# yuzhou42/disinfect-slam

Measured on AMD Instinct MI355X. Metric: TSDF integrate frames/s (640x480 depth+label, 5mm voxel), higher is better.
Workload: dtype f32

## Files before the change

### disinfect-slam_amd/csrc/tsdf_block.h

```cpp
#pragma once

#include "tsdf_device.h"

namespace tsdf {

__device__ __forceinline__ int lane_id() { return threadIdx.x & 63; }

__device__ __forceinline__ float wave_min(float v) {
#pragma unroll
  for (int o = 32; o > 0; o >>= 1) v = fminf(v, __shfl_xor(v, o, 64));
  return v;
}
__device__ __forceinline__ float wave_min_u(float v) {
  v = fminf(v, __int_as_float(__builtin_amdgcn_update_dpp(0, __float_as_int(v), 0xB1, 0xF, 0xF, false)));
  v = fminf(v, __int_as_float(__builtin_amdgcn_update_dpp(0, __float_as_int(v), 0x4E, 0xF, 0xF, false)));
  v = fminf(v, __int_as_float(__builtin_amdgcn_update_dpp(0, __float_as_int(v), 0x141, 0xF, 0xF, false)));
  v = fminf(v, __int_as_float(__builtin_amdgcn_update_dpp(0, __float_as_int(v), 0x140, 0xF, 0xF, false)));
  const int x = __float_as_int(v);
  return fminf(fminf(__int_as_float(__builtin_amdgcn_readlane(x, 0)), __int_as_float(__builtin_amdgcn_readlane(x, 16))),
               fminf(__int_as_float(__builtin_amdgcn_readlane(x, 32)), __int_as_float(__builtin_amdgcn_readlane(x, 48))));
}
__device__ __forceinline__ int wave_sum(int v) {
#pragma unroll
  for (int o = 32; o > 0; o >>= 1) v += __shfl_xor(v, o, 64);
  return v;
}
__device__ __forceinline__ int wave_incl_scan(int v) {
  const int l = lane_id();
#pragma unroll
  for (int o = 1; o < 64; o <<= 1) {
    const int n = __shfl_up(v, o, 64);
    if (l >= o) v += n;
  }
  return v;
}
template <int NW = 0>
__device__ __forceinline__ int block_excl_scan(int v, int* scratch, int* total) {
  const int w = threadIdx.x >> 6, nw = NW ? NW : blockDim.x >> 6;
  const int incl = wave_incl_scan(v);
  if (lane_id() == 63) scratch[w] = incl;
  __syncthreads();
  int before = 0, tot = 0;
#pragma unroll
  for (int i = 0; i < nw; ++i) {
// ... 210 lines not shown
```

### disinfect-slam_amd/csrc/tsdf_device.h

```cpp
#pragma once

#include <hip/hip_runtime.h>
#include <stdint.h>


namespace tsdf {

constexpr int kBlockLenBits = 3;
constexpr int kBlockLen = 8;
constexpr int kBlockVolume = 512;
constexpr int kBlockVolumeBits = 9;
constexpr int kNumBucketBits = 21;
constexpr uint32_t kNumBucket = 1u << kNumBucketBits;
constexpr uint32_t kBucketMask = kNumBucket - 1;
constexpr uint32_t kNumEntry = kNumBucket * 2;
constexpr uint32_t kEntryMask = kNumEntry - 1;
constexpr uint32_t kOccWords = kNumEntry / 64;
constexpr int kBlockBytes = kBlockVolume * 12;
constexpr int kProbOffset = kBlockVolume * 4;
constexpr int kRgbwOffset = kBlockVolume * 8;
constexpr uint32_t kNewKeyCap = 1u << 17;
constexpr int kMaxDdaSamples = 6;
constexpr int64_t kMaxOrderRange = 8192ll * 1024;
constexpr int kResolveThreads = 1024;
// ... 128 lines not shown


__device__ __forceinline__ int32_t round_quot_i(float a, float b, float rb) {
  const float q = a * rb;
  const float h = __builtin_copysignf(0.5f, q);
  const int32_t i1 = f2i(__builtin_fmaf(q, 1.0f + 0x1p-20f, h));
  const int32_t i2 = f2i(__builtin_fmaf(q, 1.0f - 0x1p-20f, h));
  if (__builtin_expect(i1 == i2 && fabsf(b) < 0x1p100f, 1)) return i1;
  return f2i(roundf(a / b));
}
__device__ __forceinline__ uint32_t round_quot_u8(float a, float b, float rb) {
  return (uint32_t)min(255, max(0, round_quot_i(a, b, rb)));
}

typedef float v2f __attribute__((ext_vector_type(2)));
__device__ __forceinline__ v2f v2(float a, float b) {
  v2f r;
  r.x = a;
  r.y = b;
  return r;
}
__device__ __forceinline__ v2f vfma(v2f a, v2f b, v2f c) { return __builtin_elementwise_fma(a, b, c); }

__device__ __forceinline__ void round_quot_i2(v2f a, v2f b, v2f rb, bool act0, bool act1,
                                              int32_t& o0, int32_t& o1) {
  const v2f q = a * rb;
  const v2f h = v2(__builtin_copysignf(0.5f, q.x), __builtin_copysignf(0.5f, q.y));
  const v2f f1 = vfma(q, v2(1.0f + 0x1p-20f, 1.0f + 0x1p-20f), h);
  const v2f f2 = vfma(q, v2(1.0f - 0x1p-20f, 1.0f - 0x1p-20f), h);
  o0 = f2i(f1.x);
  o1 = f2i(f1.y);
  if (__builtin_expect(act0 && !(o0 == f2i(f2.x) && fabsf(b.x) < 0x1p100f), 0))
    o0 = f2i(roundf(a.x / b.x));
  if (__builtin_expect(act1 && !(o1 == f2i(f2.y) && fabsf(b.y) < 0x1p100f), 0))
    o1 = f2i(roundf(a.y / b.y));
}

__device__ __forceinline__ v2f quot_const2(v2f a, float b, float rb, bool act0, bool act1) {
  const v2f q = a * rb;
  const v2f r = vfma(-q, v2(b, b), a);
  v2f o = vfma(r, v2(rb, rb), q);
  const float fa0 = fabsf(a.x), fq0 = fabsf(q.x), fa1 = fabsf(a.y), fq1 = fabsf(q.y);
  if (__builtin_expect(act0 && !(fa0 > 0x1p-60f && fa0 < 0x1p60f && fq0 > 0x1p-60f && fq0 < 0x1p60f), 0))
    o.x = a.x / b;
  if (__builtin_expect(act1 && !(fa1 > 0x1p-60f && fa1 < 0x1p60f && fq1 > 0x1p-60f && fq1 < 0x1p60f), 0))
    o.y = a.y / b;
  return o;
}

__device__ __forceinline__ void round_quot_pos2(v2f a, v2f b, v2f rb, bool act0, bool act1,
                                                int32_t& o0, int32_t& o1) {
  const v2f q = a * rb;
  const v2f f1 = vfma(q, v2(1.0f + 0x1p-20f, 1.0f + 0x1p-20f), v2(0.5f, 0.5f));
  const v2f f2 = vfma(q, v2(1.0f - 0x1p-20f, 1.0f - 0x1p-20f), v2(0.5f, 0.5f));
  o0 = f2i(f1.x);
  o1 = f2i(f1.y);
  if (__builtin_expect(act0 && o0 != f2i(f2.x), 0)) o0 = f2i(roundf(a.x / b.x));
  if (__builtin_expect(act1 && o1 != f2i(f2.y), 0)) o1 = f2i(roundf(a.y / b.y));
}

__device__ __forceinline__ v2f div_pair(v2f a, v2f b, v2f y, bool act0, bool act1) {
  const v2f e = vfma(-b, y, v2(1.0f, 1.0f));
  const v2f y1 = vfma(e, y, y);
  const v2f q = a * y1;
  const v2f r = vfma(-b, q, a);
  const v2f q1 = vfma(r, y1, q);
  const v2f r1 = vfma(-b, q1, a);
  v2f o = vfma(r1, y1, q1);
  const float fa0 = fabsf(a.x), fb0 = fabsf(b.x), fa1 = fabsf(a.y), fb1 = fabsf(b.y);
  if (__builtin_expect(act0 && !(fa0 >= 0x1p-40f && fa0 <= 0x1p40f && fb0 >= 0x1p-40f && fb0 <= 0x1p40f), 0))
    o.x = a.x / b.x;
  if (__builtin_expect(act1 && !(fa1 >= 0x1p-40f && fa1 <= 0x1p40f && fb1 >= 0x1p-40f && fb1 <= 0x1p40f), 0))
    o.y = a.y / b.y;
  return o;
}

constexpr float kSemQ[9] = {0x1.555554p-2f,  -0x1.fffffcp-3f, 0x1.999d5ap-3f,  -0x1.555b4ap-3f, 0x1.23d21ap-3f,
                            -0x1.fcf4c6p-4f, 0x1.dea282p-4f,  -0x1.d635bcp-4f, 0x1.1d8ea4p-4f};
constexpr float kSemE[6] = {0x1p-1f, 0x1.555556p-3f, 0x1.5554eap-5f, 0x1.1110e0p-7f, 0x1.6d4316p-10f,
                            0x1.a124e4p-13f};
constexpr float kSemLn2Hi = 0x1.62e4p-1f;
constexpr float kSemLn2Lo = 0x1.7f7d1cp-20f;
constexpr float kSemInvLn2 = 0x1.715476p+0f;
constexpr float kSemSqrtHalf = 0x1.6a09e6p-1f;

__device__ __forceinline__ float sem_log_reduce(float x, float& dk) {
  const bool sub = x < 0x1p-126f;
  const uint32_t ix = __float_as_uint(sub ? x * 0x1p24f : x);
  const int32_t k = (int32_t)(ix - 0x3f3504f3u) >> 23;
  dk = (float)(sub ? k - 24 : k);
  return __uint_as_float(ix - ((uint32_t)k << 23)) - 1.0f;
}
__device__ __forceinline__ v2f sem_log_core2(v2f f, v2f dk) {
  v2f q = v2(kSemQ[8], kSemQ[8]);
#pragma unroll
  for (int i = 7; i >= 0; --i) q = vfma(q, f, v2(kSemQ[i], kSemQ[i]));
// ... 211 lines not shown
  for (int i = 0; i < 8; ++i) {
    const bool v = voxel_visible(P, (int16_t)(x + ((i >> 0) & 1) * (kBlockLen - 1)),
                                 (int16_t)(y + ((i >> 1) & 1) * (kBlockLen - 1)),
                                 (int16_t)(z + ((i >> 2) & 1) * (kBlockLen - 1)));
    if (Full)
      vis = vis && v;
    else
      vis = vis || v;
  }
  return vis;
}

__device__ __forceinline__ f3 pixel_ray(const FrameParams& P, int x, int y) {
  f3 pc;
  pc.x = P.ifx * (float)x + P.icx * 1.0f;
  pc.y = P.ify * (float)y + P.icy * 1.0f;
  pc.z = 1.0f;
  return pc;
}
__device__ __forceinline__ float pixel_w_new(const FrameParams& P, float d) {
  return (1.0f - quot_const(d, P.max_depth, P.inv_max_depth)) * 4.0f;
}

}
```

### disinfect-slam_amd/csrc/tsdf_fuse.hip

```cpp
#include "tsdf_block.h"
#include "tsdf_kernels.h"
#include "tsdf_resolve.h"
#include "tsdf_ingest.h"

namespace tsdf {

__device__ __forceinline__ float comp(const float4& v, int j) {
  return j == 0 ? v.x : j == 1 ? v.y : j == 2 ? v.z : v.w;
}
__device__ __forceinline__ void setc(float4& v, int j, float f) {
  if (j == 0) v.x = f; else if (j == 1) v.y = f; else if (j == 2) v.z = f; else v.w = f;
}
__device__ __forceinline__ uint32_t compu(const uint4& v, int j) {
  return j == 0 ? v.x : j == 1 ? v.y : j == 2 ? v.z : v.w;
}
__device__ __forceinline__ void setu(uint4& v, int j, uint32_t f) {
  if (j == 0) v.x = f; else if (j == 1) v.y = f; else if (j == 2) v.z = f; else v.w = f;
}

__device__ __forceinline__ void frame_end(const EngineDev& D) {
  lds_barrier();
  if (threadIdx.x == 0) {
    D.ctr->total_visible += (unsigned long long)D.ctr->n_vis;
    D.ctr->total_updated += D.ctr->last_updated;
// ... 159 lines not shown
  const int16_t ax0 = (int16_t)(r.x << kBlockLenBits), ay = (int16_t)((r.y << kBlockLenBits) + ry),
                az = (int16_t)((r.z << kBlockLenBits) + rz);
  const float fy = (float)ay * P.voxel, fz = (float)az * P.voxel;
  const float qx = P.cq.x, qy = P.cq.y, qz = P.cq.z, qw = P.cq.w;
  const float qx_fz = qx * fz, qx_fy = qx * fy;
  float uvx = qy * fz - qz * fy;
  uvx += uvx;
  const float w_uvx = qw * uvx, qz_uvx = qz * uvx, qy_uvx = qy * uvx;
#pragma unroll
  for (int k = 0; k < 2; ++k) {
    const v2f wx = v2((float)(int16_t)(ax0 + rx0 + 2 * k), (float)(int16_t)(ax0 + rx0 + 2 * k + 1)) * P.voxel;
    v2f uvy = qz * wx - qx_fz;
    v2f uvz = qx_fy - qy * wx;
    uvy += uvy;
    uvz += uvz;
    const v2f cx = qy * uvz - qz * uvy;
    const v2f cy = qz_uvx - qx * uvz;
    const v2f cz = qx * uvy - qy_uvx;
    const v2f pcx = ((wx + w_uvx) + cx) + P.ct.x;
    const v2f pcy = ((fy + qw * uvy) + cy) + P.ct.y;
    const v2f pcz = ((fz + qw * uvz) + cz) + P.ct.z;
    const v2f hx = P.fx * pcx + P.cx * pcz;
    const v2f hy = P.fy * pcy + P.cy * pcz;
    const v2f rz = v2(__builtin_amdgcn_rcpf(pcz.x), __builtin_amdgcn_rcpf(pcz.y));
    int u0, u1, v0, v1;
    round_quot_i2(hx, pcz, rz, true, true, u0, u1);
    round_quot_i2(hy, pcz, rz, true, true, v0, v1);
    hzs[k] = pcz;
    const int uu[2] = {u0, u1}, vv[2] = {v0, v1};
#pragma unroll
    for (int e = 0; e < 2; ++e) {
      const int j = 2 * k + e;
      inb[j] = uu[e] >= 0 && uu[e] < P.W && vv[e] >= 0 && vv[e] < P.H;
      const int img = inb[j] ? vv[e] * P.W + uu[e] : 0;
      if (Raw) {
        pc[j] = (uint32_t)P.rgb[3 * img] | ((uint32_t)P.rgb[3 * img + 1] << 8) |
                ((uint32_t)P.rgb[3 * img + 2] << 16);
        px[j] = make_float4(P.depth[img], P.ht ? P.ht[img] : 1.0f, P.lt ? P.lt[img] : 1.0f,
                            __int_as_float((uu[e] & 0xFFFF) | (vv[e] << 16)));
      } else {
        px[j] = D.pixA[P.pix_off + img];
        pc[j] = D.pixC[P.pix_off + img];
      }
    }
  }
}

template <bool Raw>
__device__ __forceinline__ void update_issue(const EngineDev& D, const FrameParams& P, const VisRec& r, int lane,
                                             int hf, UpdState& S) {
// ... 28 lines not shown
    bool pf0, pf1;
    if (Raw) {
      const int w0 = __float_as_int(px[j0].w), w1 = __float_as_int(px[j1].w);
      const f3 r0 = pixel_ray(P, w0 & 0xFFFF, w0 >> 16);
      const f3 r1 = pixel_ray(P, w1 & 0xFFFF, w1 >> 16);
      rng = v2(sqrtf(dot3(r0, r0)), sqrtf(dot3(r1, r1)));
      w_new = v2(pixel_w_new(P, d.x), pixel_w_new(P, d.y));
      lnh = sem_logf2(v2(px[j0].y, px[j1].y));
      lnl = sem_logf2(v2(px[j0].z, px[j1].z));
      pf0 = sem_pixel_fast(px[j0].y, px[j0].z, d.x, P.max_depth);
      pf1 = sem_pixel_fast(px[j1].y, px[j1].z, d.y, P.max_depth);
    } else {
      rng = v2(fabsf(px[j0].y), fabsf(px[j1].y));
      pf0 = px[j0].y > 0.0f;
      pf1 = px[j1].y > 0.0f;
      lnh = v2(px[j0].z, px[j1].z);
      lnl = v2(px[j0].w, px[j1].w);
    }
    const uint32_t n0 = pc[j0], n1 = pc[j1];
    const v2f sdf = rng * (d - hzs[k]);
    const bool a0 = inb[j0] && !(d.x == 0 || d.x > P.max_depth) && sdf.x > neg_trunc;
    const bool a1 = inb[j1] && !(d.y == 0 || d.y > P.max_depth) && sdf.y > neg_trunc;
    if (a0 || a1) {
      if (!Raw) w_new = (v2(1.0f, 1.0f) - quot_const2(d, P.max_depth, P.inv_max_depth, a0, a1)) * v2(4.0f, 4.0f);
      v2f tn = quot_const2(sdf, P.trunc, P.inv_trunc, a0, a1);
      tn = v2(fminf(1.0f, tn.x), fminf(1.0f, tn.y));
      const uint32_t o0 = compu(cw, j0), o1 = compu(cw, j1);
      const v2f w_old = v2((float)(o0 >> 24), (float)(o1 >> 24));
      const v2f wc = w_old + w_new;
      const v2f iwc = v2(__builtin_amdgcn_rcpf(wc.x), __builtin_amdgcn_rcpf(wc.y));
      uint32_t c0 = 0, c1 = 0;
#pragma unroll
      for (int ch = 0; ch < 3; ++ch) {
        const v2f num = v2((float)((o0 >> (8 * ch)) & 0xFF), (float)((o1 >> (8 * ch)) & 0xFF)) * w_old +
                        v2((float)((n0 >> (8 * ch)) & 0xFF), (float)((n1 >> (8 * ch)) & 0xFF)) * w_new;
        int32_t r0, r1;
        round_quot_pos2(num, wc, iwc, a0, a1, r0, r1);
        c0 |= (uint32_t)min(255, r0) << (8 * ch);
        c1 |= (uint32_t)min(255, r1) << (8 * ch);
      }
      const v2f tnum = v2(comp(ts, j0), comp(ts, j1)) * w_old + tn * w_new;
      const v2f tq = div_pair(tnum, wc, iwc, a0, a1);
      const v2f wr = wc + v2(0x1.fffffep-2f, 0x1.fffffep-2f);
      c0 |= weight_round_cap(wr.x, 40u) << 24;
      c1 |= weight_round_cap(wr.y, 40u) << 24;
      wn[j0] = w_new.x;
      wn[j1] = w_new.y;
      if (a0) {
        setc(ts, j0, tq.x);
        setu(cw, j0, c0);
      }
      if (a1) {
        setc(ts, j1, tq.y);
        setu(cw, j1, c1);
      }
      upd_mask |= (a0 ? 1 << j0 : 0) | (a1 ? 1 << j1 : 0);
    }
    lnh2[k] = lnh;
    lnl2[k] = lnl;
    pfast |= (pf0 ? 1 << j0 : 0) | (pf1 ? 1 << j1 : 0);
    mn = fminf(mn, fminf(fabsf(comp(ts, j0)), fabsf(comp(ts, j1))));
  }
  __builtin_amdgcn_sched_barrier(0);
  {
    v2f pn2[2], pv2[2];
#pragma unroll
    for (int k = 0; k < 2; ++k) {
      const int j0 = 2 * k, j1 = 2 * k + 1;
// ... 65 lines not shown
  const int bd = __popcll(m) - 1;
  const int ofs = b - __builtin_amdgcn_readlane(bst, bd);
  return (size_t)bd * nblocks + (size_t)__builtin_amdgcn_readfirstlane(ofs);
}
__device__ __forceinline__ size_t band_find(const EngineDev& D, int bst, int lane, int b) {
  return band_find_n(D.nblocks, bst, lane, b);
}

#ifndef TSDF_INTEGRATE_WAVES
#define TSDF_INTEGRATE_WAVES 6
#endif
template <bool Graph, bool Raw>
__device__ __forceinline__ bool integrate_body(const EngineDev& D, const FrameParams& Pv,
                                               const FrameArgs* __restrict__ A, int nint, DeleteLds& L,
                                               int narrive = 0, const ViewFuse* F = nullptr) {
  FrameParams P = Graph ? A->P : Pv;
  if (Graph && A->cands_out) {
    P.tail = kTailPack;
    P.slot = A->cands_out;
    P.slot_cap = A->cand_cap;
  } else if (Graph) {
    P.tail = kTailResolve;
  }
  __shared__ float s_min[4];
  __shared__ int s_upd[4];
  __shared__ int s_last;
  __shared__ int s_ncand, s_ovf;
  __shared__ VisRec s_cand[kIntegrateCandBuf];
  const int lane = lane_id();
  const int wave = __builtin_amdgcn_readfirstlane(threadIdx.x >> 6);
  const int pair = wave >> 1, hf = wave & 1;
  int nvis = 0;
  const int bst = band_starts(D, lane, &nvis);
  const int nband = nvis;
  nvis += D.ctr->n_fresh;
  const int g = blockIdx.x & 7, ngrp = nint >> 3;
  int my_upd = 0;
  if (threadIdx.x == 0) {
    s_ncand = 0;
    s_ovf = 0;
  }
  TSDF_STAMP(D, 3, 0);
  if (blockIdx.x == 0 && threadIdx.x == 0) st_co(&D.arrive[kArrStart], (unsigned long long)__builtin_amdgcn_s_memrealtime());
  const int npairs = (nvis + 1) >> 1;
  const int p_lo = (int)(((long long)npairs * g) >> 3), p_hi = (int)(((long long)npairs * (g + 1)) >> 3);
  for (int pp = p_lo + (blockIdx.x >> 3); pp < p_hi; pp += ngrp) {
    const int b = 2 * pp + pair;
    float mn = __builtin_nanf("");
    VisRec r{};
    if (b < nvis) {
      if (b >= nband) {
        r = D.fresh_vis[b - nband];
      } else {
        r = D.vis[band_find(D, bst, lane, b)];
      }
      update_block<Raw>(D, P, r, lane, hf, mn, my_upd);
    }
    mn = wave_min_u(mn);
    if (lane == 0) s_min[wave] = mn;
    lds_barrier();
    if (hf == 0 && lane == 0 && b < nvis) {
      const float m2 = fminf(s_min[wave], s_min[wave + 1]);
      if (m2 >= 0.9f) {
        const int k = atomicAdd(&s_ncand, 1);
        if (k < kIntegrateCandBuf) {
          s_cand[k] = r;
        } else {
          const int kg = atomicAdd(D.ncand, 1);
          st_rec_co(&D.cand[kg], r);
          s_ovf = 1;
        }
      }
    }
    lds_barrier();
  }
  const int tot = wave_sum(my_upd);
  if (lane == 0) s_upd[wave] = tot;
  lds_barrier();
  const unsigned long long wg_upd = (unsigned long long)(s_upd[0] + s_upd[1] + s_upd[2] + s_upd[3]);
  const int nc = min(s_ncand, kIntegrateCandBuf);
  if (wave == 0 && nc > 0) {
    int k0 = 0;
    if (lane == 0) k0 = atomicAdd(D.ncand, nc);
    k0 = __shfl(k0, 0, 64);
    if (lane < nc) st_rec_co(&D.cand[k0 + lane], s_cand[lane]);
  }
// ... 287 lines not shown
    D.ctr->lock_epoch = epoch0 + 2u;
    D.ctr->free_count = free0 + nrel - na;
    D.ctr->last_deleted = nrel;
    D.ctr->total_deleted = tot_del + (unsigned long long)nrel;
    D.ctr->resolve_delete_ticks = ticks_del + (tick1 - tick0);
    D.ctr->resolve_alloc_ticks = ticks_alloc + (tick2 - tick1);
    st_co(&D.ctr->n_fresh, na);
    st_co(&D.ctr->nk_count, 0);
    D.ctr->last_alloc = na;
    D.ctr->last_new_keys = na;
    D.ctr->total_alloc = tot_alloc + (unsigned long long)na;
  }
  TSDF_STAMP(D, 1, 5);
  return true;
}

struct PipeUpdLds {
  int upd[4], vis[4];
  int ncand;
  VisRec cand[kIntegrateCandBuf];
  VisRec def[kPipeDefer];
  VisRec list[kPipeList];
  int n, ndef;
  float pmin[2 * kPipeList];
  int pdone[kPipeList];
  uint32_t fb;
};
union FrameLds {
  DeleteLds del;
  IngestLds<1024> ing;
  HeadLds head;
  PipeUpdLds upd;
};

__device__ __forceinline__ void merge_cands_inbox(const EngineDev& D, VisRec* cand, int32_t* ncand, const ShardRec* __restrict__ cands_in,
                                  int cap, int nshard, int* s_base);

__device__ __forceinline__ void pipe_head(const EngineDev& D, const FrameParams& Pu, const PipeArgs& A, FrameLds& U) {
  __shared__ int s_base[kMaxShards + 1];
  const int t = threadIdx.x;
  bool fast = false;
  if (A.has_carve && A.has_alloc && !A.cands_in && !A.cands_out && !resolve_fast_off() && !head_fast_off()) {
    fast = head_fast(D, A, U.head);
    if (!fast) lds_barrier();
  }
  if (A.has_carve) {
    const uint32_t f = A.fid_carve;
// ... 80 lines not shown
  bool carved_known = false;
  if (kind == 0) {
    bst = band_starts_p(D.band + (size_t)(fb % 3u) * kBands * kBandStride, lane, &nvis);
    nband = nvis;
    if (A.fresh_ready) nvis += D.ctr->n_fresh;
    const int g = wi & 7, npairs = (nvis + 1) >> 1;
    p = (int)(((long long)npairs * g) >> 3) + (wi >> 3);
    p_hi = (int)(((long long)npairs * (g + 1)) >> 3);
    pstep = A.nint >> 3;
  } else {
    wait_tag(D.pipe + kPipeAlloc + (blockIdx.x & 7) * 16, A.tag, &D.ctr->status);
    nvis = ld_co(&D.ctr->n_fresh);
    p = wi;
    p_hi = (nvis + 1) >> 1;
    pstep = kPipeFreshWG;
  }
  const bool chk = A.has_carve && kind == 0;
  const uint32_t* ct = D.ctag + (size_t)(fc & 1u) * D.nblocks;
  int my_upd = 0, my_vis = 0, ndef = 0;
  bool def_done = false;
  const bool fresh_co = kind != 0;
  int& s_n = L.n;
  int& s_ndef = L.ndef;
  float* s_pmin = L.pmin;
  int* s_pdone = L.pdone;
  uint32_t& s_fb = L.fb;
  if (t0) s_fb = fb;
  const unsigned long long lt_mask = (1ull << lane) - 1ull;
  if (t0) s_ndef = 0;
  for (;;) {
    int n = 0;
    lds_barrier();
    if (p < p_hi) {
      const int npr = min((p_hi - p + pstep - 1) / pstep, kPipeList / 2);
      if (wave == 0) {
        const int b = 2 * (p + (lane >> 1) * pstep) + (lane & 1);
        const bool valid = lane < 2 * npr && b < nvis;
        int bd = 0, bs = 0;
#pragma unroll
        for (int k = 1; k < kBands; ++k) {
          const int sk = __builtin_amdgcn_readlane(bst, k);
          if (b >= sk) {
            bd = k;
            bs = sk;
          }
        }
        VisRec r{};
// ... 41 lines not shown
        s_pdone[lane] = 0;
        if (lane == 0) s_n = __popcll(tm);
      }
      def_done = true;
    } else {
      break;
    }
    lds_barrier();
    n = s_n;
#ifdef TSDF_DIAG_STAMPS
    if (t0 && D.dbg && blockIdx.x < (unsigned)kDiagMaxWg) {
      unsigned long long* q = D.dbg + ((size_t)8 * kDiagMaxWg + blockIdx.x) * kDiagStamps;
      const unsigned long long tnow = __builtin_amdgcn_s_memrealtime();
      if (q[5] == 0ull) q[3] = tnow;
      q[4] = tnow;
      q[5] += (unsigned long long)n + 1ull;
    }
#endif
    for (int k = pair; k < n; k += 2) {
      const VisRec r = s_list[k];
      float mn = __builtin_nanf("");
      update_block<false>(D, P, r, lane, hf, mn, my_upd);
      my_vis += hf == 0 ? 1 : 0;
      mn = wave_min_u(mn);
      if (lane == 0) {
        s_pmin[2 * k + hf] = mn;
        __builtin_amdgcn_fence(__ATOMIC_RELEASE, "workgroup", "local");
        if (atomicAdd(&s_pdone[k], 1) == 1) {
          __builtin_amdgcn_fence(__ATOMIC_ACQUIRE, "workgroup", "local");
          const float m2 = fminf(mn, s_pmin[2 * k + (hf ^ 1)]);
          if (m2 >= 0.9f) {
            const uint32_t f = s_fb;
            D.ctag[(size_t)(f & 1u) * D.nblocks + r.idx] = f;
            const int kc = atomicAdd(&s_ncand, 1);
            if (kc < kIntegrateCandBuf) {
              s_cand[kc] = r;
            } else {
              const int kg = atomicAdd(ncand, 1);
              if (kg < D.cand_cap) st_rec_co(&cand[kg], r);
              else atomicOr(&D.ctr->status, 16u);
            }
          }
        }
      }
    }
  }
  const int tot = wave_sum(my_upd);
  if (lane == 0) {
    s_upd[wave] = tot;
    s_vis[wave] = my_vis;
  }
  lds_barrier();
  const int nc = min(s_ncand, kIntegrateCandBuf);
  if (wave == 0 && nc > 0) {
// ... 181 lines not shown
```

### disinfect-slam_amd/csrc/tsdf_selfcheck.hip

```cpp
#include <hip/hip_runtime.h>

#include <cstdint>
#include <cstdio>

#include "tsdf_device.h"

using namespace tsdf;

namespace {

__device__ __forceinline__ uint32_t pcg(uint32_t v) {
  const uint32_t s = v * 747796405u + 2891336453u;
  const uint32_t w = ((s >> ((s >> 28u) + 4u)) ^ s) * 277803737u;
  return (w >> 22u) ^ w;
}

__device__ __forceinline__ bool same_bits(float a, float b) {
  return __float_as_uint(a) == __float_as_uint(b) || (a != a && b != b);
}

__global__ void k_quot_const(float b, float rb, uint32_t lo, uint32_t hi,
                             unsigned long long* bad, uint32_t* first) {
  const uint64_t n = (uint64_t)hi - lo;
  for (uint64_t i = blockIdx.x * (uint64_t)blockDim.x + threadIdx.x; i < n;
       i += (uint64_t)gridDim.x * blockDim.x) {
    const uint32_t bits = lo + (uint32_t)i;
    const float a = __uint_as_float(bits);
// ... 180 lines not shown
  if (err != hipSuccess) {
    std::fprintf(stderr, "tsdf_selfcheck: %s\n", hipGetErrorString(err));
    return -2;
  }
  if (hipMemcpy(&h, d, sizeof(Out), hipMemcpyDeviceToHost) != hipSuccess) return -1;
  (void)hipFree(d);
  *bad = h.bad;
  *first = h.first;
  return 0;
}

Out* start() {
  Out* d = nullptr;
  hipError_t err = hipMalloc(&d, sizeof(Out));
  Out h{0ull, 0xFFFFFFFFu};
  if (err == hipSuccess) err = hipMemcpy(d, &h, sizeof(Out), hipMemcpyHostToDevice);
  if (err != hipSuccess) {
    std::fprintf(stderr, "tsdf_selfcheck: %s\n", hipGetErrorString(err));
    return nullptr;
  }
  return d;
}

}

extern "C" {

int tsdf_selfcheck_quot_const(float b, uint32_t lo, uint32_t hi, unsigned long long* bad,
                              uint32_t* first) {
  Out* d = start();
  if (!d) return -1;
  const float rb = 1.0f / b;
  hipLaunchKernelGGL(k_quot_const, dim3(8192), dim3(256), 0, 0, b, rb, lo, hi, &d->bad, &d->first);
  return finish(d, bad, first);
}

int tsdf_selfcheck_round_quot(uint32_t seed, uint64_t n, float bmin, float bmax, float qmax,
                              unsigned long long* bad, uint32_t* first) {
  Out* d = start();
  if (!d) return -1;
  hipLaunchKernelGGL(k_round_quot, dim3(8192), dim3(256), 0, 0, seed, n, bmin, bmax, qmax, &d->bad,
                     &d->first);
  return finish(d, bad, first);
}

int tsdf_selfcheck_quot_cmp(uint32_t seed, uint64_t n, float bmin, float bmax, float c,
// ... 31 lines not shown
}

int tsdf_selfcheck_convert(uint32_t lo, uint32_t hi, unsigned long long* bad, uint32_t* first) {
  Out* d = start();
  if (!d) return -1;
  hipLaunchKernelGGL(k_convert, dim3(8192), dim3(256), 0, 0, lo, hi, &d->bad, &d->first);
  return finish(d, bad, first);
}

int tsdf_selfcheck_sem_digest(int kind, uint64_t lo, uint64_t hi, unsigned long long* digest) {
  unsigned long long* d = nullptr;
  if (hipMalloc(&d, sizeof(*d)) != hipSuccess || hipMemset(d, 0, sizeof(*d)) != hipSuccess) return -1;
  hipLaunchKernelGGL(k_sem_digest, dim3(4096), dim3(256), 0, 0, kind, lo, hi, d);
  hipError_t err = hipGetLastError();
  if (err == hipSuccess) err = hipMemcpy(digest, d, sizeof(*d), hipMemcpyDeviceToHost);
  (void)hipFree(d);
  if (err != hipSuccess) {
    std::fprintf(stderr, "tsdf_selfcheck: %s\n", hipGetErrorString(err));
    return -2;
  }
  return 0;
}

}
```

Measured before the change: 24880.

## Replace wave-min carve test with ballots and merge cold fallback branches

The per-wave float min reduction (DPP plus readlanes) used for the carve decision becomes two ballots packed into bit flags. In the pipelined kernel these flags are OR-ed into the pair-completion atomic, which removes the LDS pmin array and its fences. The projection and voxel-update math is refactored so that all rare slow-path division fallbacks share a single branch per voxel pair rather than one branch per operation, cutting divergent branches in the hot loop. New selfcheck kernels verify that the ballot decision and the fused fallbacks match the reference.

```diff
diff --git a/disinfect-slam_amd/csrc/tsdf_block.h b/disinfect-slam_amd/csrc/tsdf_block.h
--- a/disinfect-slam_amd/csrc/tsdf_block.h
+++ b/disinfect-slam_amd/csrc/tsdf_block.h
@@ -11,15 +11,13 @@
   for (int o = 32; o > 0; o >>= 1) v = fminf(v, __shfl_xor(v, o, 64));
   return v;
 }
-__device__ __forceinline__ float wave_min_u(float v) {
-  v = fminf(v, __int_as_float(__builtin_amdgcn_update_dpp(0, __float_as_int(v), 0xB1, 0xF, 0xF, false)));
-  v = fminf(v, __int_as_float(__builtin_amdgcn_update_dpp(0, __float_as_int(v), 0x4E, 0xF, 0xF, false)));
-  v = fminf(v, __int_as_float(__builtin_amdgcn_update_dpp(0, __float_as_int(v), 0x141, 0xF, 0xF, false)));
-  v = fminf(v, __int_as_float(__builtin_amdgcn_update_dpp(0, __float_as_int(v), 0x140, 0xF, 0xF, false)));
-  const int x = __float_as_int(v);
-  return fminf(fminf(__int_as_float(__builtin_amdgcn_readlane(x, 0)), __int_as_float(__builtin_amdgcn_readlane(x, 16))),
-               fminf(__int_as_float(__builtin_amdgcn_readlane(x, 32)), __int_as_float(__builtin_amdgcn_readlane(x, 48))));
-}
+__device__ __forceinline__ uint32_t carve_bits(float mn) {
+  const bool num = __ballot(mn == mn) != 0ull;
+  const bool low = __ballot(mn < 0.9f) != 0ull;
+  return (num ? 1u << 8 : 0u) | (low ? 1u << 16 : 0u);
+}
+__device__ __forceinline__ bool carve_decide(uint32_t bits) { return (bits & (1u << 8)) != 0u && (bits & (1u << 16)) == 0u; }
+
 __device__ __forceinline__ int wave_sum(int v) {
 #pragma unroll
   for (int o = 32; o > 0; o >>= 1) v += __shfl_xor(v, o, 64);
diff --git a/disinfect-slam_amd/csrc/tsdf_device.h b/disinfect-slam_amd/csrc/tsdf_device.h
--- a/disinfect-slam_amd/csrc/tsdf_device.h
+++ b/disinfect-slam_amd/csrc/tsdf_device.h
@@ -174,7 +174,7 @@
 }
 __device__ __forceinline__ v2f vfma(v2f a, v2f b, v2f c) { return __builtin_elementwise_fma(a, b, c); }
 
-__device__ __forceinline__ void round_quot_i2(v2f a, v2f b, v2f rb, bool act0, bool act1,
+__device__ __forceinline__ void round_quot_i2_ff(v2f a, v2f b, v2f rb, bool act0, bool act1, bool& cold0, bool& cold1,
                                               int32_t& o0, int32_t& o1) {
   const v2f q = a * rb;
   const v2f h = v2(__builtin_copysignf(0.5f, q.x), __builtin_copysignf(0.5f, q.y));
@@ -182,48 +182,77 @@
   const v2f f2 = vfma(q, v2(1.0f - 0x1p-20f, 1.0f - 0x1p-20f), h);
   o0 = f2i(f1.x);
   o1 = f2i(f1.y);
-  if (__builtin_expect(act0 && !(o0 == f2i(f2.x) && fabsf(b.x) < 0x1p100f), 0))
-    o0 = f2i(roundf(a.x / b.x));
-  if (__builtin_expect(act1 && !(o1 == f2i(f2.y) && fabsf(b.y) < 0x1p100f), 0))
-    o1 = f2i(roundf(a.y / b.y));
-}
-
-__device__ __forceinline__ v2f quot_const2(v2f a, float b, float rb, bool act0, bool act1) {
+  const bool c0 = act0 && !(o0 == f2i(f2.x) && fabsf(b.x) < 0x1p100f);
+  const bool c1 = act1 && !(o1 == f2i(f2.y) && fabsf(b.y) < 0x1p100f);
+  cold0 |= c0;
+  cold1 |= c1;
+}
+
+__device__ __forceinline__ v2f quot_const2_ff(v2f a, float b, float rb, bool act0, bool act1, bool& cold0, bool& cold1) {
   const v2f q = a * rb;
   const v2f r = vfma(-q, v2(b, b), a);
-  v2f o = vfma(r, v2(rb, rb), q);
+  const v2f o = vfma(r, v2(rb, rb), q);
   const float fa0 = fabsf(a.x), fq0 = fabsf(q.x), fa1 = fabsf(a.y), fq1 = fabsf(q.y);
-  if (__builtin_expect(act0 && !(fa0 > 0x1p-60f && fa0 < 0x1p60f && fq0 > 0x1p-60f && fq0 < 0x1p60f), 0))
-    o.x = a.x / b;
-  if (__builtin_expect(act1 && !(fa1 > 0x1p-60f && fa1 < 0x1p60f && fq1 > 0x1p-60f && fq1 < 0x1p60f), 0))
-    o.y = a.y / b;
+  const bool c0 = act0 && !(fa0 > 0x1p-60f && fa0 < 0x1p60f && fq0 > 0x1p-60f && fq0 < 0x1p60f);
+  const bool c1 = act1 && !(fa1 > 0x1p-60f && fa1 < 0x1p60f && fq1 > 0x1p-60f && fq1 < 0x1p60f);
+  cold0 |= c0;
+  cold1 |= c1;
   return o;
 }
 
-__device__ __forceinline__ void round_quot_pos2(v2f a, v2f b, v2f rb, bool act0, bool act1,
+__device__ __forceinline__ void round_quot_pos2_ff(v2f a, v2f b, v2f rb, bool act0, bool act1, bool& cold0, bool& cold1,
                                                 int32_t& o0, int32_t& o1) {
   const v2f q = a * rb;
   const v2f f1 = vfma(q, v2(1.0f + 0x1p-20f, 1.0f + 0x1p-20f), v2(0.5f, 0.5f));
   const v2f f2 = vfma(q, v2(1.0f - 0x1p-20f, 1.0f - 0x1p-20f), v2(0.5f, 0.5f));
   o0 = f2i(f1.x);
   o1 = f2i(f1.y);
-  if (__builtin_expect(act0 && o0 != f2i(f2.x), 0)) o0 = f2i(roundf(a.x / b.x));
-  if (__builtin_expect(act1 && o1 != f2i(f2.y), 0)) o1 = f2i(roundf(a.y / b.y));
-}
-
-__device__ __forceinline__ v2f div_pair(v2f a, v2f b, v2f y, bool act0, bool act1) {
+  const bool c0 = act0 && o0 != f2i(f2.x);
+  const bool c1 = act1 && o1 != f2i(f2.y);
+  cold0 |= c0;
+  cold1 |= c1;
+}
+
+__device__ __forceinline__ v2f div_pair_ff(v2f a, v2f b, v2f y, bool act0, bool act1, bool& cold0, bool& cold1) {
   const v2f e = vfma(-b, y, v2(1.0f, 1.0f));
   const v2f y1 = vfma(e, y, y);
   const v2f q = a * y1;
   const v2f r = vfma(-b, q, a);
   const v2f q1 = vfma(r, y1, q);
   const v2f r1 = vfma(-b, q1, a);
-  v2f o = vfma(r1, y1, q1);
+  const v2f o = vfma(r1, y1, q1);
   const float fa0 = fabsf(a.x), fb0 = fabsf(b.x), fa1 = fabsf(a.y), fb1 = fabsf(b.y);
-  if (__builtin_expect(act0 && !(fa0 >= 0x1p-40f && fa0 <= 0x1p40f && fb0 >= 0x1p-40f && fb0 <= 0x1p40f), 0))
-    o.x = a.x / b.x;
-  if (__builtin_expect(act1 && !(fa1 >= 0x1p-40f && fa1 <= 0x1p40f && fb1 >= 0x1p-40f && fb1 <= 0x1p40f), 0))
-    o.y = a.y / b.y;
+  const bool c0 = act0 && !(fa0 >= 0x1p-40f && fa0 <= 0x1p40f && fb0 >= 0x1p-40f && fb0 <= 0x1p40f);
+  const bool c1 = act1 && !(fa1 >= 0x1p-40f && fa1 <= 0x1p40f && fb1 >= 0x1p-40f && fb1 <= 0x1p40f);
+  cold0 |= c0;
+  cold1 |= c1;
+  return o;
+}
+
+__device__ __forceinline__ void round_quot_i2(v2f a, v2f b, v2f rb, bool act0, bool act1, int32_t& o0, int32_t& o1) {
+  bool c0 = false, c1 = false;
+  round_quot_i2_ff(a, b, rb, act0, act1, c0, c1, o0, o1);
+  if (__builtin_expect(c0, 0)) o0 = f2i(roundf(a.x / b.x));
+  if (__builtin_expect(c1, 0)) o1 = f2i(roundf(a.y / b.y));
+}
+__device__ __forceinline__ v2f quot_const2(v2f a, float b, float rb, bool act0, bool act1) {
+  bool c0 = false, c1 = false;
+  v2f o = quot_const2_ff(a, b, rb, act0, act1, c0, c1);
+  if (__builtin_expect(c0, 0)) o.x = a.x / b;
+  if (__builtin_expect(c1, 0)) o.y = a.y / b;
+  return o;
+}
+__device__ __forceinline__ void round_quot_pos2(v2f a, v2f b, v2f rb, bool act0, bool act1, int32_t& o0, int32_t& o1) {
+  bool c0 = false, c1 = false;
+  round_quot_pos2_ff(a, b, rb, act0, act1, c0, c1, o0, o1);
+  if (__builtin_expect(c0, 0)) o0 = f2i(roundf(a.x / b.x));
+  if (__builtin_expect(c1, 0)) o1 = f2i(roundf(a.y / b.y));
+}
+__device__ __forceinline__ v2f div_pair(v2f a, v2f b, v2f y, bool act0, bool act1) {
+  bool c0 = false, c1 = false;
+  v2f o = div_pair_ff(a, b, y, act0, act1, c0, c1);
+  if (__builtin_expect(c0, 0)) o.x = a.x / b.x;
+  if (__builtin_expect(c1, 0)) o.y = a.y / b.y;
   return o;
 }
 
@@ -481,4 +510,88 @@
   return (1.0f - quot_const(d, P.max_depth, P.inv_max_depth)) * 4.0f;
 }
 
-}
+
+__device__ __forceinline__ void project_pair(v2f hx, v2f hy, v2f pcz, int& u0, int& u1, int& v0, int& v1, bool& cold0,
+                                             bool& cold1) {
+  const v2f rz = v2(__builtin_amdgcn_rcpf(pcz.x), __builtin_amdgcn_rcpf(pcz.y));
+  bool c0 = false, c1 = false;
+  round_quot_i2_ff(hx, pcz, rz, true, true, c0, c1, u0, u1);
+  round_quot_i2_ff(hy, pcz, rz, true, true, c0, c1, v0, v1);
+  if (__builtin_expect(c0 || c1, 0)) {
+    if (c0) {
+      u0 = f2i(roundf(hx.x / pcz.x));
+      v0 = f2i(roundf(hy.x / pcz.x));
+    }
+    if (c1) {
+      u1 = f2i(roundf(hx.y / pcz.y));
+      v1 = f2i(roundf(hy.y / pcz.y));
+    }
+  }
+  cold0 = c0;
+  cold1 = c1;
+}
+
+__device__ __forceinline__ float averages_exact(uint32_t o, uint32_t n, float w_old, float w_new, float wc, float t_old,
+                                                float tn, uint32_t& c) {
+  c = 0;
+#pragma unroll
+  for (int ch = 0; ch < 3; ++ch) {
+    const float num = (float)((o >> (8 * ch)) & 0xFF) * w_old + (float)((n >> (8 * ch)) & 0xFF) * w_new;
+    c |= (uint32_t)min(255, f2i(roundf(num / wc))) << (8 * ch);
+  }
+  return (t_old * w_old + tn * w_new) / wc;
+}
+
+template <bool Raw>
+__device__ __forceinline__ void update_pair(const FrameParams& P, v2f d, v2f sdf, bool a0, bool a1, uint32_t o0, uint32_t o1,
+                                            uint32_t n0, uint32_t n1, v2f t_old, v2f& w_new, v2f& tq, uint32_t& c0,
+                                            uint32_t& c1, bool& cold0, bool& cold1) {
+  bool ca0 = false, ca1 = false;
+  v2f dq = v2(0.f, 0.f);
+  if (!Raw) dq = quot_const2_ff(d, P.max_depth, P.inv_max_depth, true, true, ca0, ca1);
+  v2f tn = quot_const2_ff(sdf, P.trunc, P.inv_trunc, true, true, ca0, ca1);
+  ca0 = ca0 && a0;
+  ca1 = ca1 && a1;
+  if (__builtin_expect(ca0 || ca1, 0)) {
+    if (ca0) {
+      if (!Raw) dq.x = d.x / P.max_depth;
+      tn.x = sdf.x / P.trunc;
+    }
+    if (ca1) {
+      if (!Raw) dq.y = d.y / P.max_depth;
+      tn.y = sdf.y / P.trunc;
+    }
+  }
+  if (!Raw) w_new = (v2(1.0f, 1.0f) - dq) * v2(4.0f, 4.0f);
+  tn = v2(fminf(1.0f, tn.x), fminf(1.0f, tn.y));
+  const v2f w_old = v2((float)(o0 >> 24), (float)(o1 >> 24));
+  const v2f wc = w_old + w_new;
+  const v2f iwc = v2(__builtin_amdgcn_rcpf(wc.x), __builtin_amdgcn_rcpf(wc.y));
+  c0 = 0;
+  c1 = 0;
+  bool cb0 = false, cb1 = false;
+#pragma unroll
+  for (int ch = 0; ch < 3; ++ch) {
+    const v2f num = v2((float)((o0 >> (8 * ch)) & 0xFF), (float)((o1 >> (8 * ch)) & 0xFF)) * w_old +
+                    v2((float)((n0 >> (8 * ch)) & 0xFF), (float)((n1 >> (8 * ch)) & 0xFF)) * w_new;
+    int32_t r0, r1;
+    round_quot_pos2_ff(num, wc, iwc, true, true, cb0, cb1, r0, r1);
+    c0 |= (uint32_t)min(255, r0) << (8 * ch);
+    c1 |= (uint32_t)min(255, r1) << (8 * ch);
+  }
+  const v2f tnum = t_old * w_old + tn * w_new;
+  tq = div_pair_ff(tnum, wc, iwc, true, true, cb0, cb1);
+  cb0 = cb0 && a0;
+  cb1 = cb1 && a1;
+  if (__builtin_expect(cb0 || cb1, 0)) {
+    if (cb0) tq.x = averages_exact(o0, n0, w_old.x, w_new.x, wc.x, t_old.x, tn.x, c0);
+    if (cb1) tq.y = averages_exact(o1, n1, w_old.y, w_new.y, wc.y, t_old.y, tn.y, c1);
+  }
+  const v2f wr = wc + v2(0x1.fffffep-2f, 0x1.fffffep-2f);
+  c0 |= weight_round_cap(wr.x, 40u) << 24;
+  c1 |= weight_round_cap(wr.y, 40u) << 24;
+  cold0 = ca0 || cb0;
+  cold1 = ca1 || cb1;
+}
+
+}
diff --git a/disinfect-slam_amd/csrc/tsdf_fuse.hip b/disinfect-slam_amd/csrc/tsdf_fuse.hip
--- a/disinfect-slam_amd/csrc/tsdf_fuse.hip
+++ b/disinfect-slam_amd/csrc/tsdf_fuse.hip
@@ -205,10 +205,9 @@
     const v2f pcz = ((fz + qw * uvz) + cz) + P.ct.z;
     const v2f hx = P.fx * pcx + P.cx * pcz;
     const v2f hy = P.fy * pcy + P.cy * pcz;
-    const v2f rz = v2(__builtin_amdgcn_rcpf(pcz.x), __builtin_amdgcn_rcpf(pcz.y));
     int u0, u1, v0, v1;
-    round_quot_i2(hx, pcz, rz, true, true, u0, u1);
-    round_quot_i2(hy, pcz, rz, true, true, v0, v1);
+    bool cold0, cold1;
+    project_pair(hx, hy, pcz, u0, u1, v0, v1, cold0, cold1);
     hzs[k] = pcz;
     const int uu[2] = {u0, u1}, vv[2] = {v0, v1};
 #pragma unroll
@@ -283,28 +282,12 @@
     const bool a0 = inb[j0] && !(d.x == 0 || d.x > P.max_depth) && sdf.x > neg_trunc;
     const bool a1 = inb[j1] && !(d.y == 0 || d.y > P.max_depth) && sdf.y > neg_trunc;
     if (a0 || a1) {
-      if (!Raw) w_new = (v2(1.0f, 1.0f) - quot_const2(d, P.max_depth, P.inv_max_depth, a0, a1)) * v2(4.0f, 4.0f);
-      v2f tn = quot_const2(sdf, P.trunc, P.inv_trunc, a0, a1);
-      tn = v2(fminf(1.0f, tn.x), fminf(1.0f, tn.y));
       const uint32_t o0 = compu(cw, j0), o1 = compu(cw, j1);
-      const v2f w_old = v2((float)(o0 >> 24), (float)(o1 >> 24));
-      const v2f wc = w_old + w_new;
-      const v2f iwc = v2(__builtin_amdgcn_rcpf(wc.x), __builtin_amdgcn_rcpf(wc.y));
-      uint32_t c0 = 0, c1 = 0;
-#pragma unroll
-      for (int ch = 0; ch < 3; ++ch) {
-        const v2f num = v2((float)((o0 >> (8 * ch)) & 0xFF), (float)((o1 >> (8 * ch)) & 0xFF)) * w_old +
-                        v2((float)((n0 >> (8 * ch)) & 0xFF), (float)((n1 >> (8 * ch)) & 0xFF)) * w_new;
-        int32_t r0, r1;
-        round_quot_pos2(num, wc, iwc, a0, a1, r0, r1);
-        c0 |= (uint32_t)min(255, r0) << (8 * ch);
-        c1 |= (uint32_t)min(255, r1) << (8 * ch);
-      }
-      const v2f tnum = v2(comp(ts, j0), comp(ts, j1)) * w_old + tn * w_new;
-      const v2f tq = div_pair(tnum, wc, iwc, a0, a1);
-      const v2f wr = wc + v2(0x1.fffffep-2f, 0x1.fffffep-2f);
-      c0 |= weight_round_cap(wr.x, 40u) << 24;
-      c1 |= weight_round_cap(wr.y, 40u) << 24;
+      uint32_t c0, c1;
+      v2f tq;
+      bool cold0, cold1;
+      update_pair<Raw>(P, d, sdf, a0, a1, o0, o1, n0, n1, v2(comp(ts, j0), comp(ts, j1)), w_new, tq, c0, c1, cold0,
+                       cold1);
       wn[j0] = w_new.x;
       wn[j1] = w_new.y;
       if (a0) {
@@ -416,7 +399,7 @@
   } else if (Graph) {
     P.tail = kTailResolve;
   }
-  __shared__ float s_min[4];
+  __shared__ uint32_t s_cb[4];
   __shared__ int s_upd[4];
   __shared__ int s_last;
   __shared__ int s_ncand, s_ovf;
@@ -450,12 +433,11 @@
       }
       update_block<Raw>(D, P, r, lane, hf, mn, my_upd);
     }
-    mn = wave_min_u(mn);
-    if (lane == 0) s_min[wave] = mn;
+    const uint32_t cb = carve_bits(mn);
+    if (lane == 0) s_cb[wave] = cb;
     lds_barrier();
     if (hf == 0 && lane == 0 && b < nvis) {
-      const float m2 = fminf(s_min[wave], s_min[wave + 1]);
-      if (m2 >= 0.9f) {
+      if (carve_decide(s_cb[wave] | s_cb[wave + 1])) {
         const int k = atomicAdd(&s_ncand, 1);
         if (k < kIntegrateCandBuf) {
           s_cand[k] = r;
@@ -789,7 +771,6 @@
   VisRec def[kPipeDefer];
   VisRec list[kPipeList];
   int n, ndef;
-  float pmin[2 * kPipeList];
   int pdone[kPipeList];
   uint32_t fb;
 };
@@ -916,7 +897,6 @@
   const bool fresh_co = kind != 0;
   int& s_n = L.n;
   int& s_ndef = L.ndef;
-  float* s_pmin = L.pmin;
   int* s_pdone = L.pdone;
   uint32_t& s_fb = L.fb;
   if (t0) s_fb = fb;
@@ -1004,14 +984,11 @@
       float mn = __builtin_nanf("");
       update_block<false>(D, P, r, lane, hf, mn, my_upd);
       my_vis += hf == 0 ? 1 : 0;
-      mn = wave_min_u(mn);
+      const uint32_t cb = carve_bits(mn);
       if (lane == 0) {
-        s_pmin[2 * k + hf] = mn;
-        __builtin_amdgcn_fence(__ATOMIC_RELEASE, "workgroup", "local");
-        if (atomicAdd(&s_pdone[k], 1) == 1) {
-          __builtin_amdgcn_fence(__ATOMIC_ACQUIRE, "workgroup", "local");
-          const float m2 = fminf(mn, s_pmin[2 * k + (hf ^ 1)]);
-          if (m2 >= 0.9f) {
+        const uint32_t prev = (uint32_t)atomicAdd(&s_pdone[k], (int)(1u | cb));
+        if (prev & 1u) {
+          if (carve_decide(cb | prev)) {
             const uint32_t f = s_fb;
             D.ctag[(size_t)(f & 1u) * D.nblocks + r.idx] = f;
             const int kc = atomicAdd(&s_ncand, 1);
diff --git a/disinfect-slam_amd/csrc/tsdf_selfcheck.hip b/disinfect-slam_amd/csrc/tsdf_selfcheck.hip
--- a/disinfect-slam_amd/csrc/tsdf_selfcheck.hip
+++ b/disinfect-slam_amd/csrc/tsdf_selfcheck.hip
@@ -3,6 +3,7 @@
 #include <cstdint>
 #include <cstdio>
 
+#include "tsdf_block.h"
 #include "tsdf_device.h"
 
 using namespace tsdf;
@@ -229,6 +230,189 @@
   return d;
 }
 
+__device__ __forceinline__ float carve_palette(uint32_t h, bool high_only) {
+  const float t = 0.9f;
+  const float below = __uint_as_float(__float_as_uint(t) - 1u), above = __uint_as_float(__float_as_uint(t) + 1u);
+  const float rnd = (h >> 8) * 0x1p-23f - 1.0f;
+  if (high_only) {
+    switch (h & 7u) {
+      case 0: return t;
+      case 1: return -t;
+      case 2: return above;
+      case 3: return 1.0f;
+      case 4: return -1.0f;
+      case 5: return __builtin_inff();
+      case 6: return -above;
+      default: return 0.9f + 0.1f * fabsf(rnd);
+    }
+  }
+  switch (h & 15u) {
+    case 0: return t;
+    case 1: return -t;
+    case 2: return below;
+    case 3: return -below;
+    case 4: return above;
+    case 5: return 0.0f;
+    case 6: return -0.0f;
+    case 7: return 1.0f;
+    case 8: return __builtin_nanf("");
+    case 9: return -__builtin_nanf("");
+    case 10: return __builtin_inff();
+    case 11: return 0x1p-149f;
+    default: return rnd;
+  }
+}
+__global__ void k_carve(uint32_t seed, uint32_t nblocks, unsigned long long* out) {
+  const int lane = threadIdx.x & 63;
+  const uint32_t wave = (blockIdx.x * blockDim.x + threadIdx.x) >> 6, nwaves = (gridDim.x * blockDim.x) >> 6;
+  const float nan = __builtin_nanf("");
+  for (uint32_t b = wave; b < nblocks; b += nwaves) {
+    const uint32_t mode = b % 6u, hb = pcg(b ^ seed);
+    float mn[2];
+    bool any_num = false;
+#pragma unroll
+    for (int hf = 0; hf < 2; ++hf) {
+      float m = nan;
+#pragma unroll
+      for (int j = 0; j < 4; ++j) {
+        const uint32_t vox = (uint32_t)(hf * 256 + lane * 4 + j), h = pcg(pcg(hb + vox) ^ 0x85ebca6bu);
+        float v;
+        if (mode == 0) v = nan;
+        else if (mode == 1) v = (h & 0x300u) ? carve_palette(h, true) : nan;
+        else if (mode == 2) v = vox == (hb >> 4) % 512u ? carve_palette(h, false) : nan;
+        else if (mode == 3) v = carve_palette(h, false);
+        else if (mode == 4) v = vox == (hb >> 4) % 512u ? __uint_as_float(__float_as_uint(0.9f) - 1u) : carve_palette(h, true);
+        else v = hf == (int)(hb & 1u) ? nan : carve_palette(h, (hb & 2u) != 0u);
+        m = fminf(m, fabsf(v));
+        any_num = any_num || v == v;
+      }
+      mn[hf] = m;
+    }
+    const bool ref = fminf(wave_min(mn[0]), wave_min(mn[1])) >= 0.9f;
+    const bool got = carve_decide(carve_bits(mn[0]) | carve_bits(mn[1]));
+    const bool all_nan = __ballot(any_num) == 0ull;
+    if (lane == 0) {
+      if (ref != got) atomicAdd(&out[0], 1ull);
+      atomicAdd(&out[got ? 1 : 2], 1ull);
+      if (all_nan && got) atomicAdd(&out[3], 1ull);
+    }
+  }
+}
+
+__device__ __forceinline__ float ulps(float x, int k) { return __uint_as_float(__float_as_uint(x) + (uint32_t)k); }
+__device__ __forceinline__ float edge_value(uint32_t h, float e0, float e1) {
+  const float e = (h & 1u) ? e0 : e1;
+  float v;
+  switch ((h >> 1) & 7u) {
+    case 0: v = e; break;
+    case 1: v = ulps(e, 1); break;
+    case 2: v = ulps(e, -1); break;
+    case 3: v = 0.0f; break;
+    case 4: v = __builtin_inff(); break;
+    case 5: v = __builtin_nanf(""); break;
+    case 6: v = e * 0.5f; break;
+    default: v = e * 2.0f; break;
+  }
+  return (h & 16u) ? -v : v;
+}
+struct VoxIn {
+  float d, sdf, t_old;
+  uint32_t o, n;
+  bool act;
+};
+__device__ __forceinline__ VoxIn gen_voxel(uint32_t h, int mode, float max_depth, float trunc) {
+  const uint32_t h1 = pcg(h), h2 = pcg(h1 ^ 0x9e3779b9u), h3 = pcg(h2 + 0x85ebca6bu);
+  VoxIn v;
+  v.n = h1 & 0xFFFFFFu;
+  v.o = (h2 & 0xFFFFFFu) | ((h3 % 41u) << 24);
+  v.act = (h3 >> 8 & 7u) != 0u;
+  v.d = 0.3f + 3.6f * ((h1 >> 8) * 0x1p-24f) * (max_depth * 0.25f);
+  v.sdf = trunc * (4.0f * ((h2 >> 8) * 0x1p-24f) - 1.0f);
+  v.t_old = (h3 >> 8) * 0x1p-23f - 1.0f;
+  if (mode == 1) {
+    const uint32_t w = 1u + (h3 >> 11) % 3u;
+    v.o = (v.o & 0xFFFFFFu) | (w << 24);
+    v.d = ulps(max_depth * (1.0f - (float)w * 0.25f), (int)((h3 >> 16) % 5u) - 2);
+  } else if (mode == 2) {
+    switch ((h3 >> 11) & 3u) {
+      case 0: v.sdf = edge_value(h1 >> 3, 0x1p-60f, 0x1p60f); break;
+      case 1: v.t_old = edge_value(h1 >> 3, 0x1p-40f, 0x1p40f); v.d = max_depth; v.o = (v.o & 0xFFFFFFu) | (1u << 24); break;
+      case 2: v.d = fabsf(edge_value((h1 >> 3) & ~8u, 0x1p-60f, max_depth)); break;
+      default: v.d = max_depth; if (h1 & 8u) v.o &= 0xFFFFFFu; break;
+    }
+  }
+  v.act = v.act && !(v.d == 0 || v.d > max_depth) && v.sdf > -trunc;
+  return v;
+}
+__global__ void k_update_pair(uint32_t seed, uint64_t n, int mode, float max_depth, float inv_max_depth, float trunc,
+                              float inv_trunc, unsigned long long* out) {
+  FrameParams P{};
+  P.max_depth = max_depth;
+  P.inv_max_depth = inv_max_depth;
+  P.trunc = trunc;
+  P.inv_trunc = inv_trunc;
+  unsigned long long bad = 0, act = 0, cold = 0, pbad = 0, pix = 0, pcold = 0;
+  for (uint64_t i = blockIdx.x * (uint64_t)blockDim.x + threadIdx.x; i < n; i += (uint64_t)gridDim.x * blockDim.x) {
+    const uint32_t h = pcg((uint32_t)i ^ seed) + (uint32_t)(i >> 32);
+    const VoxIn x = gen_voxel(h, mode, max_depth, trunc), y = gen_voxel(h ^ 0xA5A5A5A5u, mode, max_depth, trunc);
+    v2f w_new = v2(0.f, 0.f), tq;
+    uint32_t c0, c1;
+    bool f0, f1;
+    update_pair<false>(P, v2(x.d, y.d), v2(x.sdf, y.sdf), x.act, y.act, x.o, y.o, x.n, y.n, v2(x.t_old, y.t_old), w_new,
+                       tq, c0, c1, f0, f1);
+#pragma unroll
+    for (int e = 0; e < 2; ++e) {
+      const VoxIn& v = e ? y : x;
+      if (!v.act) continue;
+      const float rw = (1.0f - v.d / max_depth) * 4.0f;
+      const float tn = fminf(1.0f, v.sdf / trunc);
+      const float w_old = (float)(v.o >> 24), wc = w_old + rw;
+      uint32_t rc = 0;
+#pragma unroll
+      for (int ch = 0; ch < 3; ++ch) {
+        const float num = (float)((v.o >> (8 * ch)) & 0xFF) * w_old + (float)((v.n >> (8 * ch)) & 0xFF) * rw;
+        rc |= (uint32_t)min(255, f2i(roundf(num / wc))) << (8 * ch);
+      }
+      rc |= weight_round_cap(wc + 0x1.fffffep-2f, 40u) << 24;
+      const float rt = (v.t_old * w_old + tn * rw) / wc;
+      ++act;
+      cold += (e ? f1 : f0) ? 1 : 0;
+      if (!same_bits(e ? w_new.y : w_new.x, rw) || !same_bits(e ? tq.y : tq.x, rt) || (e ? c1 : c0) != rc) ++bad;
+    }
+    const uint32_t g0 = pcg(h ^ 0x51ed270bu), g1 = pcg(g0 + 1u), g2 = pcg(g1 + 2u), g3 = pcg(g2 + 3u);
+    float z[2], ax[2], ay[2];
+#pragma unroll
+    for (int e = 0; e < 2; ++e) {
+      const uint32_t a = e ? g1 : g0, b = e ? g3 : g2;
+      z[e] = 0.05f + 9.95f * ((a >> 8) * 0x1p-24f);
+      ax[e] = ((b >> 8) * 0x1p-23f - 0.5f) * 700.0f * z[e];
+      ay[e] = ((pcg(b) >> 8) * 0x1p-23f - 0.5f) * 500.0f * z[e];
+      if (mode == 1) {
+        ax[e] = ulps((floorf(ax[e] / z[e]) + 0.5f) * z[e], (int)(a & 7u) - 4);
+        if (b & 1u) ay[e] = ulps((floorf(ay[e] / z[e]) - 0.5f) * z[e], (int)((a >> 3) & 7u) - 4);
+      } else if (mode == 2 && (a & 3u) == 0u) {
+        z[e] = edge_value(b, 0x1p100f, 0x1p-100f);
+      }
+    }
+    int u0, u1, v0, v1;
+    bool q0, q1;
+    project_pair(v2(ax[0], ax[1]), v2(ay[0], ay[1]), v2(z[0], z[1]), u0, u1, v0, v1, q0, q1);
+#pragma unroll
+    for (int e = 0; e < 2; ++e) {
+      const int ru = f2i(roundf(ax[e] / z[e])), rv = f2i(roundf(ay[e] / z[e]));
+      ++pix;
+      pcold += (e ? q1 : q0) ? 1 : 0;
+      if ((e ? u1 : u0) != ru || (e ? v1 : v0) != rv) ++pbad;
+    }
+  }
+  if (bad) atomicAdd(&out[0], bad);
+  atomicAdd(&out[1], act);
+  atomicAdd(&out[2], cold);
+  if (pbad) atomicAdd(&out[3], pbad);
+  atomicAdd(&out[4], pix);
+  atomicAdd(&out[5], pcold);
+}
+
 }
 
 extern "C" {
@@ -306,4 +490,33 @@
   return 0;
 }
 
-}
+int tsdf_selfcheck_carve(uint32_t seed, uint32_t nblocks, unsigned long long* out) {
+  unsigned long long* d = nullptr;
+  if (hipMalloc(&d, 4 * sizeof(*d)) != hipSuccess || hipMemset(d, 0, 4 * sizeof(*d)) != hipSuccess) return -1;
+  hipLaunchKernelGGL(k_carve, dim3(1024), dim3(256), 0, 0, seed, nblocks, d);
+  hipError_t err = hipGetLastError();
+  if (err == hipSuccess) err = hipMemcpy(out, d, 4 * sizeof(*d), hipMemcpyDeviceToHost);
+  (void)hipFree(d);
+  if (err != hipSuccess) {
+    std::fprintf(stderr, "tsdf_selfcheck: %s\n", hipGetErrorString(err));
+    return -2;
+  }
+  return 0;
+}
+
+int tsdf_selfcheck_update(uint32_t seed, uint64_t n, int mode, float max_depth, float trunc, unsigned long long* out) {
+  unsigned long long* d = nullptr;
+  if (hipMalloc(&d, 6 * sizeof(*d)) != hipSuccess || hipMemset(d, 0, 6 * sizeof(*d)) != hipSuccess) return -1;
+  hipLaunchKernelGGL(k_update_pair, dim3(2048), dim3(256), 0, 0, seed, n, mode, max_depth, 1.0f / max_depth, trunc,
+                     1.0f / trunc, d);
+  hipError_t err = hipGetLastError();
+  if (err == hipSuccess) err = hipMemcpy(out, d, 6 * sizeof(*d), hipMemcpyDeviceToHost);
+  (void)hipFree(d);
+  if (err != hipSuccess) {
+    std::fprintf(stderr, "tsdf_selfcheck: %s\n", hipGetErrorString(err));
+    return -2;
+  }
+  return 0;
+}
+
+}
```

Result: no change. 25130 (median of 6 runs) (+1.0%).
